# yashsmehta/visreps

Hardware: AMD Instinct MI355X
Metric: end-to-end RSA eval sec (extract→RDM→1000-bootstrap Spearman), N=10k stimuli (lower is better)
Workload: dtype bf16x3-split Gram, fp32 accumulate (|dSpearman| < 1e-5 vs fp64 RDMs: tests/test_benchsize.py) / exact int ranks, fp64 statistic

## Files before the change

### visreps_amd/csrc/rdm.hip

```cpp
#include <cstdlib>
#include <cstring>

#include "internal.h"

namespace vr {

typedef float f32x4 __attribute__((ext_vector_type(4)));
typedef float f32x16 __attribute__((ext_vector_type(16)));

constexpr int RSTAT_BS = 256;

__device__ inline double block_sum_f64(double v, double* lds) {
  for (int o = 32; o > 0; o >>= 1) v += __shfl_down(v, o, 64);
  const int lane = threadIdx.x & 63, wid = threadIdx.x >> 6;
  if (lane == 0) lds[wid] = v;
  __syncthreads();
  double s = 0;
  if (threadIdx.x == 0) {
    for (int w = 0; w < RSTAT_BS / 64; ++w) s += lds[w];
    lds[RSTAT_BS / 64] = s;
  }
  __syncthreads();
  s = lds[RSTAT_BS / 64];
  __syncthreads();
// ... 790 lines not shown
        aH[m] = __builtin_bit_cast(bf16x8, *reinterpret_cast<const u32x4*>(ar));
        aL[m] = __builtin_bit_cast(bf16x8, *reinterpret_cast<const u32x4*>(ar + 32));
      }
#pragma unroll
      for (int nn = 0; nn < 2; ++nn) {
        const uint16_t* br = Bs + (wc * 64 + nn * 32 + l32) * SROW + t * 16 + h * 8;
        bH[nn] = __builtin_bit_cast(bf16x8, *reinterpret_cast<const u32x4*>(br));
        bL[nn] = __builtin_bit_cast(bf16x8, *reinterpret_cast<const u32x4*>(br + 32));
      }
#pragma unroll
      for (int m = 0; m < 4; ++m)
#pragma unroll
        for (int nn = 0; nn < 2; ++nn)
          acc[m][nn] = __builtin_amdgcn_mfma_f32_32x32x16_bf16(aH[m], bH[nn], acc[m][nn], 0, 0, 0);
#pragma unroll
      for (int m = 0; m < 4; ++m)
#pragma unroll
        for (int nn = 0; nn < 2; ++nn)
          acc[m][nn] = __builtin_amdgcn_mfma_f32_32x32x16_bf16(aH[m], bL[nn], acc[m][nn], 0, 0, 0);
#pragma unroll
      for (int m = 0; m < 4; ++m)
#pragma unroll
        for (int nn = 0; nn < 2; ++nn)
          acc[m][nn] = __builtin_amdgcn_mfma_f32_32x32x16_bf16(aL[m], bH[nn], acc[m][nn], 0, 0, 0);
    }
    if (more) {
      uint16_t* nxt = lds + (cur ^ 1) * 2 * W_STAGE;
      store_rec_w(nxt, ga);
      if (!diag) store_rec_w(nxt + W_STAGE, gb);
    }
    if (P.flush && more && (kt + 1) % P.flush == 0) {
      gram_flush<WT>(acc, P.fbuf + (size_t)blockIdx.x * WT * WT, wr * 128, wc * 64, kt + 1 == P.flush);
    }
    __syncthreads();
  }
  if (P.flush && ns > P.flush) gram_unflush<WT>(acc, P.fbuf + (size_t)blockIdx.x * WT * WT, wr * 128, wc * 64);
  gram_store_w(P, acc, row0, col0, diag);
}

constexpr int P_PANEL = WT * 64;
constexpr int P_SLOT = 2 * P_PANEL;
constexpr int P_SLOTS = 4;
constexpr int P_AHEAD = P_SLOTS - 1;
static_assert(P_AHEAD == 3, "the counted waits of gram3p_step / gram3p_loop assume 4 slots");

__device__ inline void p_issue(const GramParams& P, char* panel, int64_t row0, int q) {
  const int lane = threadIdx.x & 63, wid = threadIdx.x >> 6;
  const int64_t st = q >> 1;
  const int t = q & 1;
#pragma unroll
  for (int i = 0; i < 2; ++i) {
    const int rbase = (wid * 2 + i) * 16;
    const int r = rbase + (lane >> 2);
    const int j = (lane & 3) ^ ((r >> 2) & 3);
    const int off = ((j & 2) << 5) + 32 * t + ((j & 1) << 4);
    const char* src = reinterpret_cast<const char*>(P.planes) + ((row0 + r) * P.nstage + st) * 128 + off;
    __builtin_amdgcn_global_load_lds(src, panel + rbase * 64, 16, 0, 0);
  }
}

__device__ inline bf16x8 p_frag(const char* panel, int row, int j) {
  return __builtin_bit_cast(bf16x8, *reinterpret_cast<const u32x4*>(panel + row * 64 + ((j ^ ((row >> 2) & 3)) << 4)));
}

template <int N>
__device__ inline void p_wait() {
  asm volatile("s_waitcnt vmcnt(%0)" ::"n"(N) : "memory");
}

struct PFrag {
  bf16x8 aH[4], aL[4], bH[2], bL[2];
};

__device__ inline void p_read(const char* As, const char* Bs, PFrag& f) {
  const int lane = threadIdx.x & 63, wid = threadIdx.x >> 6;
  const int wr = wid >> 2, wc = wid & 3, h = lane >> 5, l32 = lane & 31;
#pragma unroll
  for (int m = 0; m < 4; ++m) {
    const int r = wr * 128 + m * 32 + l32;
    f.aH[m] = p_frag(As, r, h);
    f.aL[m] = p_frag(As, r, 2 + h);
  }
#pragma unroll
  for (int nn = 0; nn < 2; ++nn) {
    const int r = wc * 64 + nn * 32 + l32;
    f.bH[nn] = p_frag(Bs, r, h);
    f.bL[nn] = p_frag(Bs, r, 2 + h);
  }
}

__device__ inline void p_mfma(const PFrag& f, f32x16 (&acc)[4][2]) {
#pragma unroll
  for (int m = 0; m < 4; ++m)
#pragma unroll
    for (int nn = 0; nn < 2; ++nn)
      acc[m][nn] = __builtin_amdgcn_mfma_f32_32x32x16_bf16(f.aH[m], f.bH[nn], acc[m][nn], 0, 0, 0);
#pragma unroll
  for (int m = 0; m < 4; ++m)
#pragma unroll
    for (int nn = 0; nn < 2; ++nn)
      acc[m][nn] = __builtin_amdgcn_mfma_f32_32x32x16_bf16(f.aH[m], f.bL[nn], acc[m][nn], 0, 0, 0);
#pragma unroll
  for (int m = 0; m < 4; ++m)
#pragma unroll
    for (int nn = 0; nn < 2; ++nn)
      acc[m][nn] = __builtin_amdgcn_mfma_f32_32x32x16_bf16(f.aL[m], f.bH[nn], acc[m][nn], 0, 0, 0);
}

template <bool DIAG>
__device__ inline void gram3p_step(const GramParams& P, char* lds, int64_t row0, int64_t col0, int q, int Q,
                                   const PFrag& cur, PFrag& nxt, f32x16 (&acc)[4][2]) {
  constexpr int PER = DIAG ? 2 : 4;
  if (q + 1 < Q) {
    const int left = Q - 2 - q;
    if (left >= 1)
      p_wait<PER>();
    else
      p_wait<0>();
    __builtin_amdgcn_s_barrier();
    if (q + P_AHEAD < Q) {
      char* slot = lds + ((q + P_AHEAD) % P_SLOTS) * P_SLOT;
      p_issue(P, slot, row0, q + P_AHEAD);
      if (!DIAG) p_issue(P, slot + P_PANEL, col0, q + P_AHEAD);
    }
    const char* As = lds + ((q + 1) % P_SLOTS) * P_SLOT;
    p_read(As, DIAG ? As : As + P_PANEL, nxt);
  }
  p_mfma(cur, acc);
  if (P.flush && (q & 1) && q + 1 < Q && ((q >> 1) + 1) % P.flush == 0) {
    const int wid = threadIdx.x >> 6;
    gram_flush<WT>(acc, P.fbuf + (size_t)blockIdx.x * WT * WT, (wid >> 2) * 128, (wid & 3) * 64,
                   (q >> 1) + 1 == P.flush);
  }
}

template <bool DIAG>
__device__ inline void gram3p_loop(const GramParams& P, char* lds, int64_t row0, int64_t col0, int ns,
                                   f32x16 (&acc)[4][2]) {
  const int Q = 2 * ns;
  constexpr int PER = DIAG ? 2 : 4;
  for (int q = 0; q < P_AHEAD && q < Q; ++q) {
    char* slot = lds + q * P_SLOT;
    p_issue(P, slot, row0, q);
    if (!DIAG) p_issue(P, slot + P_PANEL, col0, q);
  }
  if (Q > 2)
    p_wait<2 * PER>();
  else if (Q > 1)
    p_wait<PER>();
  else
    p_wait<0>();
  __builtin_amdgcn_s_barrier();
  PFrag f0, f1;
  p_read(lds, DIAG ? lds : lds + P_PANEL, f0);
  for (int q = 0; q < Q; q += 2) {
    gram3p_step<DIAG>(P, lds, row0, col0, q, Q, f0, f1, acc);
    gram3p_step<DIAG>(P, lds, row0, col0, q + 1, Q, f1, f0, acc);
  }
}

__device__ inline void gram_partial_w(const GramParams& P, f32x16 (&acc)[4][2], int split, int ltile) {
  const int lane = threadIdx.x & 63, wid = threadIdx.x >> 6;
  const int wr = wid >> 2, wc = wid & 3, h = lane >> 5, l32 = lane & 31;
  float* out = P.partial + ((int64_t)split * P.tile_count + ltile) * (WT * WT);
#pragma unroll
  for (int m = 0; m < 4; ++m)
#pragma unroll
    for (int nn = 0; nn < 2; ++nn) {
      const int lj = wc * 64 + nn * 32 + l32;
#pragma unroll
      for (int r = 0; r < 16; ++r) {
        const int li = wr * 128 + m * 32 + (r & 3) + 8 * (r >> 2) + 4 * h;
        out[li * WT + lj] = acc[m][nn][r];
      }
    }
}

__global__ __launch_bounds__(W_THREADS, 1) void k_gram3p(GramParams P) {
  __shared__ __attribute__((aligned(16))) char lds[P_SLOTS * P_SLOT];
  const int id = P.blk0 + (int)xcd_remap(blockIdx.x, (uint32_t)gridDim.x);
  const int split = id / P.tile_count, ltile = id % P.tile_count;
  int bi, bj;
  band_tile(ltile, P.tile0, P.tile_count, P.T, bi, bj);
  const bool diag = (bi == bj);
  const int64_t row0 = (int64_t)bi * WT, col0 = (int64_t)bj * WT;
  const int lane = threadIdx.x & 63, wid = threadIdx.x >> 6;
  const int wr = wid >> 2, wc = wid & 3;
  (void)lane;
  const int64_t sper = P.kslice / GK;
  const int64_t st0 = (int64_t)split * sper;
  const int ns = (int)(P.nstage - st0 < sper ? P.nstage - st0 : sper);
  GramParams S = P;
  S.planes = P.planes + st0 * 64;
  f32x16 acc[4][2];
#pragma unroll
  for (int a = 0; a < 4; ++a)
#pragma unroll
    for (int b = 0; b < 2; ++b)
#pragma unroll
      for (int e = 0; e < 16; ++e) acc[a][b][e] = 0.f;
  if (diag)
    gram3p_loop<true>(S, lds, row0, col0, ns, acc);
  else
    gram3p_loop<false>(S, lds, row0, col0, ns, acc);
  if (P.flush && ns > P.flush)
    gram_unflush<WT>(acc, P.fbuf + (size_t)blockIdx.x * WT * WT, wr * 128, wc * 64);
  if (P.splits == 1)
    gram_store_w(P, acc, row0, col0, diag);
  else
    gram_partial_w(P, acc, split, ltile);
}

__global__ __launch_bounds__(256) void k_gram_reduce_w(GramParams P) {
  __shared__ float tr[32][33];
  const int ltile = blockIdx.x;
  int bi, bj;
  band_tile(ltile, P.tile0, P.tile_count, P.T, bi, bj);
  const bool diag = (bi == bj);
  const int64_t row0 = (int64_t)bi * WT, col0 = (int64_t)bj * WT;
  const int tx = threadIdx.x & 31, ty = threadIdx.x >> 5;
  const int si0 = blockIdx.y * 32;
  for (int sj0 = 0; sj0 < WT; sj0 += 32) {
    for (int yy = ty; yy < 32; yy += 8) {
      const int li = si0 + yy, lj = sj0 + tx;
      const int pi = (diag && li > lj) ? lj : li, pj = (diag && li > lj) ? li : lj;
      float g = 0.f;
      for (int s = 0; s < P.splits; ++s)
        g += P.partial[((int64_t)s * P.tile_count + ltile) * (WT * WT) + pi * WT + pj];
      const int64_t i = row0 + li, j = col0 + lj;
      const float sI = (i < P.n) ? P.stdv[i] : 1.f, sJ = (j < P.n) ? P.stdv[j] : 1.f;
      const float v = rdm_value(g, i, j, P, sI, sJ);
      if (i < P.n && j < P.n) P.rdm[i * P.ldr + j] = v;
      tr[yy][tx] = v;
    }
    __syncthreads();
    if (!diag) {
      for (int yy = ty; yy < 32; yy += 8) {
        const int64_t j = col0 + sj0 + yy, i = row0 + si0 + tx;
        if (i < P.n && j < P.n) P.rdm[j * P.ldr + i] = tr[tx][yy];
      }
    }
    __syncthreads();
  }
}

constexpr int E_HALF = 128 * 128;
constexpr int E_STAGE = 4 * E_HALF;

__device__ inline uint32_t e_issue_off(const GramParams& P, int k) {
  const int lane = threadIdx.x & 63, wid = threadIdx.x >> 6;
  const int rr = wid * 16 + k * 8 + (lane >> 3);
  const int c = (lane & 7) ^ ((rr >> 1) & 7);
  return (uint32_t)rr * (uint32_t)P.nstage * 128u + (uint32_t)c * 16u;
}
__device__ inline void e_issue(const GramParams& P, char* sb, int h, int64_t row0, int64_t col0, int64_t st,
                               const uint32_t (&io)[2]) {
  const int wid = threadIdx.x >> 6;
  const int64_t rbase = (h < 2 ? row0 : col0) + (h & 1) * 128;
  const char* base = reinterpret_cast<const char*>(P.planes) + (rbase * P.nstage + st) * 128;
  char* half = sb + h * E_HALF;
#pragma unroll
  for (int k = 0; k < 2; ++k) {
    uint32_t off = io[k];
    asm volatile("" : "+v"(off));
    __builtin_amdgcn_global_load_lds(base + off, half + (wid * 16 + k * 8) * 128, 16, 0, 0);
  }
}

struct EFragA {
  bf16x8 hi[4], lo[4];
};
struct EFragB {
  bf16x8 hi[2], lo[2];
};

struct ELane {
  uint32_t hi, lo;
};
__device__ inline ELane e_lane() {
  const int lane = threadIdx.x & 63, g = lane >> 4, l16 = lane & 15, swz = (l16 >> 1) & 7;
  return ELane{(uint32_t)(l16 * 128 + ((g ^ swz) << 4)), (uint32_t)(l16 * 128 + (((4 + g) ^ swz) << 4))};
}
__device__ inline void e_read_a(const char* half, int r0, const ELane& o, EFragA& f) {
  uint32_t ohi = o.hi, olo = o.lo;
  asm volatile("" : "+v"(ohi), "+v"(olo));
#pragma unroll
  for (int m = 0; m < 4; ++m) {
    const char* row = half + (r0 + m * 16) * 128;
    f.hi[m] = __builtin_bit_cast(bf16x8, *reinterpret_cast<const u32x4*>(row + ohi));
    f.lo[m] = __builtin_bit_cast(bf16x8, *reinterpret_cast<const u32x4*>(row + olo));
  }
}
__device__ inline void e_read_b(const char* half, int r0, const ELane& o, EFragB& f) {
  uint32_t ohi = o.hi, olo = o.lo;
  asm volatile("" : "+v"(ohi), "+v"(olo));
#pragma unroll
  for (int n = 0; n < 2; ++n) {
    const char* row = half + (r0 + n * 16) * 128;
    f.hi[n] = __builtin_bit_cast(bf16x8, *reinterpret_cast<const u32x4*>(row + ohi));
    f.lo[n] = __builtin_bit_cast(bf16x8, *reinterpret_cast<const u32x4*>(row + olo));
  }
}

template <int MA, int NB, bool ONE>
__device__ inline void e_mfma(const EFragA& a, const EFragB& b, f32x4 (&acc)[8][4]) {
#pragma unroll
  for (int m = 0; m < 4; ++m)
#pragma unroll
    for (int n = 0; n < 2; ++n)
      acc[MA * 4 + m][NB * 2 + n] =
          __builtin_amdgcn_mfma_f32_16x16x32_bf16(a.hi[m], b.hi[n], acc[MA * 4 + m][NB * 2 + n], 0, 0, 0);
  if constexpr (ONE) {
#pragma unroll
    for (int m = 0; m < 4; ++m)
#pragma unroll
      for (int n = 0; n < 2; ++n)
        acc[MA * 4 + m][NB * 2 + n] =
            __builtin_amdgcn_mfma_f32_16x16x32_bf16(a.lo[m], b.lo[n], acc[MA * 4 + m][NB * 2 + n], 0, 0, 0);
    return;
  }
#pragma unroll
  for (int m = 0; m < 4; ++m)
#pragma unroll
    for (int n = 0; n < 2; ++n)
      acc[MA * 4 + m][NB * 2 + n] =
          __builtin_amdgcn_mfma_f32_16x16x32_bf16(a.hi[m], b.lo[n], acc[MA * 4 + m][NB * 2 + n], 0, 0, 0);
#pragma unroll
  for (int m = 0; m < 4; ++m)
#pragma unroll
    for (int n = 0; n < 2; ++n)
      acc[MA * 4 + m][NB * 2 + n] =
          __builtin_amdgcn_mfma_f32_16x16x32_bf16(a.lo[m], b.hi[n], acc[MA * 4 + m][NB * 2 + n], 0, 0, 0);
}

__device__ inline float* e_flush_base(float* buf) {
  const int lane = threadIdx.x & 63, wid = threadIdx.x >> 6;
  uint32_t off = (uint32_t)(((wid >> 2) * 128 + 4 * (lane >> 4)) * WT + (wid & 3) * 64 + (lane & 15));
  asm volatile("" : "+v"(off));
  return buf + off;
}
__device__ inline void e_flush(f32x4 (&acc)[8][4], float* buf, bool first) {
  float* b = e_flush_base(buf);
#pragma unroll
  for (int i = 0; i < 8; ++i)
#pragma unroll
    for (int j = 0; j < 4; ++j)
#pragma unroll
      for (int e = 0; e < 4; ++e) {
        float* p = b + (i * 16 + e) * WT + j * 16;
        *p = first ? acc[i][j][e] : *p + acc[i][j][e];
        acc[i][j][e] = 0.f;
      }
}
__device__ inline void e_unflush(f32x4 (&acc)[8][4], const float* buf) {
  const float* b = e_flush_base(const_cast<float*>(buf));
#pragma unroll
  for (int i = 0; i < 8; ++i)
#pragma unroll
    for (int j = 0; j < 4; ++j)
#pragma unroll
      for (int e = 0; e < 4; ++e) acc[i][j][e] += b[(i * 16 + e) * WT + j * 16];
}

template <bool ONE>
__device__ inline void e_store(const GramParams& P, f32x4 (&acc)[8][4], int64_t row0, int64_t col0, bool diag) {
  const int lane = threadIdx.x & 63, wid = threadIdx.x >> 6;
  const int wr = wid >> 2, wc = wid & 3, g = lane >> 4, l16 = lane & 15;
#pragma unroll
  for (int j4 = 0; j4 < 4; ++j4) {
    const int64_t j = col0 + wc * 64 + j4 * 16 + l16;
    const float sj = (j < P.n) ? P.stdv[j] : 1.f;
#pragma unroll
    for (int i8 = 0; i8 < 8; ++i8) {
      const int64_t ib = row0 + wr * 128 + i8 * 16 + 4 * g;
      float v[4];
#pragma unroll
      for (int e = 0; e < 4; ++e) {
        const int64_t i = ib + e;
        const float si = (i < P.n) ? P.stdv[i] : 1.f;
        v[e] = rdm_value_t<ONE>(acc[i8][j4][e], i, j, P, si, sj);
      }
      if (diag) {
#pragma unroll
        for (int e = 0; e < 4; ++e) {
          const int64_t i = ib + e;
          if (i <= j && j < P.n) {
            P.rdm[i * P.ldr + j] = v[e];
            if (i < j) P.rdm[j * P.ldr + i] = v[e];
          }
        }
        continue;
      }
#pragma unroll
      for (int e = 0; e < 4; ++e) {
        const int64_t i = ib + e;
        if (i < P.n && j < P.n) P.rdm[i * P.ldr + j] = v[e];
      }
      if (j < P.n) {
        float* dst = P.rdm + j * P.ldr + ib;
        if (P.vec && ib + 3 < P.n && ((P.ldr & 3) == 0)) {
          f32x4 w = {v[0], v[1], v[2], v[3]};
          *reinterpret_cast<f32x4*>(dst) = w;
        } else {
#pragma unroll
          for (int e = 0; e < 4; ++e)
            if (ib + e < P.n) dst[e] = v[e];
        }
      }
    }
  }
}

__device__ inline void e_barrier() {
  __builtin_amdgcn_s_barrier();
  asm volatile("" ::: "memory");
}

template <bool DIAG, bool ODD, bool ONE>
__device__ inline void e_stage(const GramParams& P, char* lds, int64_t row0, int64_t col0, int t, int ns,
                               const ELane& o, const uint32_t (&io)[2], EFragA& AX, EFragA& AY,
                               EFragB& BP, EFragB& BQ, f32x4 (&acc)[8][4]) {
  const int wid = threadIdx.x >> 6;
  const int wr = wid >> 2, wc = wid & 3;
  EFragB& B0 = ODD ? BQ : BP;
  EFragB& B1 = ODD ? BP : BQ;
  char* cur = lds + (t & 1) * E_STAGE;
  char* nxt = lds + ((t + 1) & 1) * E_STAGE;
  const int ha = wr, hb = DIAG ? (wc >> 1) : 2 + (wc >> 1);
  const int rb = (wc & 1) * 64;
  const bool more1 = t + 1 < ns, more2 = t + 2 < ns;
  e_barrier();
  if (more1) e_issue(P, nxt, 1, row0, col0, t + 1, io);
  e_read_b(cur + hb * E_HALF, rb + 32, o, B1);
  e_mfma<0, 0, ONE>(AX, B0, acc);
  e_barrier();
  if (!DIAG && more1) e_issue(P, nxt, 3, row0, col0, t + 1, io);
  e_read_a(cur + ha * E_HALF, 64, o, AY);
  e_mfma<0, 1, ONE>(AX, B1, acc);
  if (more1) {
    if (DIAG)
      p_wait<0>();
    else
      p_wait<2>();
  }
  e_barrier();
  if (!DIAG && more2) e_issue(P, cur, 2, row0, col0, t + 2, io);
  if (more1) e_read_a(nxt + ha * E_HALF, 0, o, AX);
  e_mfma<1, 1, ONE>(AY, B1, acc);
  if (!DIAG && more1) {
    if (more2)
      p_wait<2>();
    else
      p_wait<0>();
  }
  e_barrier();
  if (more2) e_issue(P, cur, 0, row0, col0, t + 2, io);
  if (more1) e_read_b(nxt + hb * E_HALF, rb, o, B1);
  e_mfma<1, 0, ONE>(AY, B0, acc);
  if (P.flush && more1 && (t + 1) % P.flush == 0) e_flush(acc, P.fbuf + (size_t)blockIdx.x * WT * WT, t + 1 == P.flush);
}

template <bool DIAG, bool ONE>
__device__ inline void e_loop(const GramParams& P, char* lds, int64_t row0, int64_t col0, int ns,
                              f32x4 (&acc)[8][4]) {
  const int wid = threadIdx.x >> 6;
  const int wr = wid >> 2, wc = wid & 3;
  const int ha = wr, hb = DIAG ? (wc >> 1) : 2 + (wc >> 1), rb = (wc & 1) * 64;
  const uint32_t io[2] = {e_issue_off(P, 0), e_issue_off(P, 1)};
  e_issue(P, lds, 0, row0, col0, 0, io);
  e_issue(P, lds, 1, row0, col0, 0, io);
  if (!DIAG) {
    e_issue(P, lds, 2, row0, col0, 0, io);
    e_issue(P, lds, 3, row0, col0, 0, io);
  }
  if (ns > 1) {
    if (!DIAG) e_issue(P, lds + E_STAGE, 2, row0, col0, 1, io);
    e_issue(P, lds + E_STAGE, 0, row0, col0, 1, io);
    if (DIAG)
      p_wait<2>();
    else
      p_wait<4>();
  } else {
    p_wait<0>();
  }
  e_barrier();
  const ELane o = e_lane();
  EFragA AX, AY;
  EFragB BP, BQ;
  e_read_a(lds + ha * E_HALF, 0, o, AX);
  e_read_b(lds + hb * E_HALF, rb, o, BP);
  for (int t = 0; t < ns; t += 2) {
    e_stage<DIAG, false, ONE>(P, lds, row0, col0, t, ns, o, io, AX, AY, BP, BQ, acc);
    if (t + 1 < ns) e_stage<DIAG, true, ONE>(P, lds, row0, col0, t + 1, ns, o, io, AX, AY, BP, BQ, acc);
  }
}

__device__ inline void e_partial(const GramParams& P, f32x4 (&acc)[8][4], int split, int ltile) {
  const int lane = threadIdx.x & 63, wid = threadIdx.x >> 6;
  const int wr = wid >> 2, wc = wid & 3, g = lane >> 4, l16 = lane & 15;
  float* out = P.partial + ((int64_t)split * P.tile_count + ltile) * (WT * WT);
#pragma unroll
  for (int i = 0; i < 8; ++i)
#pragma unroll
    for (int j = 0; j < 4; ++j)
#pragma unroll
      for (int e = 0; e < 4; ++e) out[(wr * 128 + i * 16 + 4 * g + e) * WT + wc * 64 + j * 16 + l16] = acc[i][j][e];
}

template <bool ONE>
__global__ __launch_bounds__(W_THREADS, 1) void k_gram3e(GramParams P) {
  __shared__ __attribute__((aligned(16))) char lds[2 * E_STAGE];
  const int id = P.blk0 + (int)xcd_remap(blockIdx.x, (uint32_t)gridDim.x);
  const int split = id / P.tile_count, ltile = id % P.tile_count;
  int bi, bj;
  band_tile(ltile, P.tile0, P.tile_count, P.T, bi, bj);
  const bool diag = (bi == bj);
  const int64_t row0 = (int64_t)bi * WT, col0 = (int64_t)bj * WT;
  const int64_t sper = P.kslice / GK;
  const int64_t st0 = (int64_t)split * sper;
  const int ns = (int)(P.nstage - st0 < sper ? P.nstage - st0 : sper);
  GramParams S = P;
  S.planes = P.planes + st0 * 64;
  f32x4 acc[8][4];
#pragma unroll
  for (int i = 0; i < 8; ++i)
#pragma unroll
    for (int j = 0; j < 4; ++j) acc[i][j] = f32x4{0.f, 0.f, 0.f, 0.f};
  if (diag)
    e_loop<true, ONE>(S, lds, row0, col0, ns, acc);
  else
    e_loop<false, ONE>(S, lds, row0, col0, ns, acc);
  if (P.flush && ns > P.flush) e_unflush(acc, P.fbuf + (size_t)blockIdx.x * WT * WT);
  if (P.splits == 1)
    e_store<ONE>(P, acc, row0, col0, diag);
  else
    e_partial(P, acc, split, ltile);
}

static bool env_flag(const char* name, bool dflt) {
  const char* e = getenv(name);
  return e && *e ? strcmp(e, "0") != 0 : dflt;
}

static bool gram_phased() {
  const char* e = getenv("VISREPS_GRAM_KERNEL");
  return !(e && strcmp(e, "p") == 0);
}

static bool gram_pipe() {
  const char* e = getenv("VISREPS_GRAM_PIPE");
  return !(e && strcmp(e, "0") == 0);
}

__global__ __launch_bounds__(256) void k_gram_reduce(GramParams P) {
  __shared__ float tr[32][33];
  const int ltile = blockIdx.x;
  int bi, bj;
  band_tile(ltile, P.tile0, P.tile_count, P.T, bi, bj);
  const bool diag = (bi == bj);
  const int64_t row0 = (int64_t)bi * GT, col0 = (int64_t)bj * GT;
  const int tx = threadIdx.x & 31, ty = threadIdx.x >> 5;
  for (int sb = 0; sb < (GT / 32) * (GT / 32); ++sb) {
    const int si0 = (sb / (GT / 32)) * 32, sj0 = (sb % (GT / 32)) * 32;
    for (int yy = ty; yy < 32; yy += 8) {
      const int li = si0 + yy, lj = sj0 + tx;
      float g = 0.f;
      const int pi = (diag && li > lj) ? lj : li, pj = (diag && li > lj) ? li : lj;
      for (int s = 0; s < P.splits; ++s)
        g += P.partial[((int64_t)s * P.tile_count + ltile) * (GT * GT) + pi * GT + pj];
      const int64_t i = row0 + li, j = col0 + lj;
      const float sI = (i < P.n) ? P.stdv[i] : 1.f, sJ = (j < P.n) ? P.stdv[j] : 1.f;
      const float v = rdm_value(g, i, j, P, sI, sJ);
      if (i < P.n && j < P.n) P.rdm[i * P.ldr + j] = v;
      tr[yy][tx] = v;
    }
    __syncthreads();
    if (!diag) {
      for (int yy = ty; yy < 32; yy += 8) {
        const int64_t j = col0 + sj0 + yy, i = row0 + si0 + tx;
        if (i < P.n && j < P.n) P.rdm[j * P.ldr + i] = tr[tx][yy];
      }
    }
    __syncthreads();
  }
}

static int64_t gram_tiles(int64_t n) {
  const int64_t T = (n + GT - 1) / GT;
  return T * (T + 1) / 2;
}

static void gram_geometry(int64_t n, int64_t d, int64_t count, int& T, int& ntiles,
                          int& splits, int64_t& kslice, bool fit = false) {
  T = (int)((n + GT - 1) / GT);
  ntiles = T * (T + 1) / 2;
  const int64_t kt = (d + GK - 1) / GK;
  const int target = 2 * num_cus();
  int s = 1;
  if (count < target) {
    s = fit ? (int)std::max<int64_t>(1, target / count) : (int)((target + count - 1) / count);
    const int64_t maxs = std::max<int64_t>(1, kt / 4);
    if (s > maxs) s = (int)maxs;
  }
  const int64_t per = (kt + s - 1) / s;
  kslice = per * GK;
  splits = (int)((d + kslice - 1) / kslice);
  if (splits < 1) splits = 1;
}

static bool gram_split(int64_t n, int64_t d) {
  const char* e = getenv("VISREPS_GRAM");
  if (e && strcmp(e, "fp32") == 0) return false;
  if (e && strcmp(e, "split") == 0) return true;
  return (double)n * (double)n * (double)d >= 1e10;
}

static int gram_generation(int nblk) {
  int gen = 2 * num_cus();
  if (const char* e = getenv("VISREPS_GRAM_GEN")) {
    const int v = atoi(e);
    gen = v > 0 ? v : nblk;
  }
  return std::max(1, gen);
}

static int64_t gram_tail(int64_t count) {
  const int gen = 2 * num_cus();
  if (getenv("VISREPS_GRAM_GEN") || count <= gen) return 0;
  const int64_t tail = count % gen;
  return (tail > 0 && tail <= gen / 2) ? tail : 0;
}

static size_t range_partial(int64_t n, int64_t d, int64_t count, bool fit_one = false) {
  if (count <= 0) return 0;
  int T, ntiles, splits;
  int64_t kslice;
  if (fit_one && count < 2 * num_cus()) {
    gram_geometry(n, d, count, T, ntiles, splits, kslice, true);
    return splits > 1 ? (size_t)splits * count * GT * GT : 0;
  }
  const int64_t tail = gram_tail(count);
  gram_geometry(n, d, count - tail, T, ntiles, splits, kslice);
  size_t part = splits > 1 ? (size_t)splits * (count - tail) : 0;
  if (tail > 0) {
    gram_geometry(n, d, tail, T, ntiles, splits, kslice, true);
    if (splits > 1) part = std::max(part, (size_t)splits * tail);
  }
  return part * GT * GT;
}

static int64_t tri_start(int64_t r, int64_t T) { return r * T - r * (r - 1) / 2; }

static int gram_wide_rows(int64_t n, int64_t d, bool split3) {
  if (!split3) return 0;
  if (const char* e = getenv("VISREPS_GRAM_WIDE"))
    if (strcmp(e, "0") == 0) return 0;
  const int64_t T2 = (n + WT - 1) / WT, gen = num_cus();
  const int64_t full = (T2 * (T2 + 1) / 2) / gen * gen;
  if (full < gen) return 0;
  int64_t R = 0;
  while (R + 1 <= T2 && tri_start(R + 1, T2) <= full) ++R;
  (void)d;
  return (int)R;
}

struct RangePlan {
  bool wide = false;
  int64_t s0 = 0, s1 = 0;
  int64_t r0 = 0, r_count = 0;
  int r_splits = 1;
  int64_t rem0 = 0, rem_count = 0;
  bool rem_fit = false;
};

static int wide_rem_splits(int64_t count, int64_t nstage) {
  const int64_t gen = num_cus();
  if (count <= 0 || count >= gen) return 1;
  int64_t s = gen / count;
  s = std::min<int64_t>(s, std::max<int64_t>(1, nstage / 8));
  const int64_t per = (nstage + s - 1) / s;
  return (int)((nstage + per - 1) / per);
}

static RangePlan plan_range(int64_t n, int64_t d, int64_t t0, int64_t t1, bool split3) {
  RangePlan rp;
  const int64_t total = gram_tiles(n), T = (n + GT - 1) / GT, T2 = (n + WT - 1) / WT;
  const int R = gram_wide_rows(n, d, split3);
  rp.rem0 = t0;
  rp.rem_count = t1 - t0;
  if (R == 0 || t1 <= t0) return rp;
  int64_t r0 = -1, r1 = -1;
  for (int64_t r = 0; r <= R; ++r) {
    if (tri_start(2 * r, T) == t0) r0 = r;
    if (tri_start(2 * r, T) == t1) r1 = r;
  }
  if (r0 < 0 || (t1 != total && r1 < 0)) return rp;
  const int64_t trem = tri_start(2 * (int64_t)R, T);
  rp.wide = true;
  rp.s0 = tri_start(r0, T2);
  rp.s1 = t1 == total ? tri_start(R, T2) : tri_start(r1, T2);
  rp.rem_count = 0;
  static const bool wide_rem = !(getenv("VISREPS_GRAM_WIDE_REM") && strcmp(getenv("VISREPS_GRAM_WIDE_REM"), "0") == 0);
  if (t1 == total && !wide_rem) {
    rp.rem0 = trem;
    rp.rem_count = total - trem;
    rp.rem_fit = true;
  } else if (t1 == total) {
    rp.r0 = tri_start(R, T2);
    rp.r_count = T2 * (T2 + 1) / 2 - rp.r0;
    rp.r_splits = wide_rem_splits(rp.r_count, (d + GK - 1) / GK);
  }
  return rp;
}

static int gram_flush_stages() {
  int f = 256;
  if (const char* e = getenv("VISREPS_GRAM_FLUSH")) f = atoi(e);
  return f > 0 ? f : 0;
}
static size_t gram_fbuf_floats() {
  return std::max<size_t>((size_t)2 * num_cus() * GT * GT, (size_t)num_cus() * WT * WT);
}

static size_t gram_ws(int64_t n, int64_t d, int64_t t0, int64_t t1, bool split3, void* base, float** mean,
                      float** stdv, float** partial, uint16_t** planes, float** fbuf = nullptr,
                      bool own_planes = true, uint32_t** flag = nullptr) {
  const RangePlan rp = plan_range(n, d, t0, t1, split3);
  size_t part = range_partial(n, d, rp.rem_count, rp.rem_fit);
  if (rp.r_splits > 1) part = std::max(part, (size_t)rp.r_count * rp.r_splits * WT * WT);
  Carver c(base);
  float* m = c.take<float>((size_t)n);
  float* s = c.take<float>((size_t)n);
  float* p = part ? c.take<float>(part) : nullptr;
  const int64_t prow = (n + WT - 1) / WT * WT;
  uint16_t* pl = split3 && own_planes ? c.take<uint16_t>((size_t)prow * (size_t)((d + GK - 1) / GK) * 64)
                                      : nullptr;
  const bool flush = gram_flush_stages() > 0 && (d + GK - 1) / GK > gram_flush_stages();
  float* fb = flush ? c.take<float>(gram_fbuf_floats()) : nullptr;
  uint32_t* fl = c.take<uint32_t>(64);
  if (flag) *flag = fl;
  if (fbuf) *fbuf = fb;
  if (mean) *mean = m;
  if (stdv) *stdv = s;
  if (partial) *partial = p;
  if (planes) *planes = pl;
  return c.bytes();
}

}

using namespace vr;

extern "C" {

size_t vr_rdm_pearson_workspace(int64_t n, int64_t d) {
  if (n <= 0 || d <= 0) return 256;
  return gram_ws(n, d, 0, gram_tiles(n), gram_split(n, d), nullptr, nullptr, nullptr, nullptr, nullptr);
}

size_t vr_rdm_tiles_workspace(int64_t n, int64_t d, int64_t tile_begin, int64_t tile_end) {
  if (n <= 0 || d <= 0 || tile_end <= tile_begin) return 256;
  return gram_ws(n, d, tile_begin, tile_end, gram_split(n, d), nullptr, nullptr, nullptr, nullptr,
                 nullptr);
}

int64_t vr_rdm_tile_count(int64_t n) { return n > 0 ? gram_tiles(n) : 0; }

int64_t vr_rdm_wide_rows(int64_t n, int64_t d) {
  return n > 0 && d > 0 ? gram_wide_rows(n, d, gram_split(n, d)) : 0;
}

int vr_rdm_range_aligned(int64_t n, int64_t d, int64_t tile_begin, int64_t tile_end) {
  if (n <= 0 || d <= 0 || tile_begin < 0 || tile_end > gram_tiles(n) || tile_end < tile_begin) return 0;
  if (tile_begin == tile_end) return 1;
  if (tile_begin == 0 && tile_end == gram_tiles(n)) return 1;
  return plan_range(n, d, tile_begin, tile_end, gram_split(n, d)).wide ? 1 : 0;
}

int64_t vr_rdm_tile_cost(int64_t n, int64_t tile) {
  int T = (int)((n + GT - 1) / GT), bi, bj;
  int p = (int)tile, r = 0;
  while (r + 1 < T && (int64_t)(r + 1) * T - (int64_t)(r + 1) * r / 2 <= p) ++r;
  bi = r;
  bj = r + (p - (r * T - r * (r - 1) / 2));
  const int64_t h = std::min<int64_t>(GT, n - (int64_t)bi * GT), w = std::min<int64_t>(GT, n - (int64_t)bj * GT);
  return bi == bj ? h * (h + 1) / 2 : h * w;
}

int vr_rdm_tile_rect(int64_t n, int64_t tile, int64_t* row0, int64_t* col0, int64_t* rows,
                     int64_t* cols) {
  VR_REQUIRE(n > 0 && tile >= 0 && tile < gram_tiles(n), "vr_rdm_tile_rect: tile %lld of %lld",
             (long long)tile, (long long)(n > 0 ? gram_tiles(n) : 0));
  VR_REQUIRE(row0 && col0 && rows && cols, "vr_rdm_tile_rect: null output");
  const int T = (int)((n + GT - 1) / GT);
  int p = (int)tile, r = 0;
  while (r + 1 < T && (int64_t)(r + 1) * T - (int64_t)(r + 1) * r / 2 <= p) ++r;
  const int bi = r, bj = r + (p - (r * T - r * (r - 1) / 2));
  *row0 = (int64_t)bi * GT;
  *col0 = (int64_t)bj * GT;
  *rows = std::min<int64_t>(GT, n - *row0);
  *cols = std::min<int64_t>(GT, n - *col0);
  return VR_OK;
}

int vr_row_stats_f32(const float* X, int64_t n, int64_t d, int64_t ldx, float* mean,
                     float* stdv, float correction, void* stream) {
  VR_REQUIRE(n >= 0 && d > 0 && ldx >= d, "vr_row_stats_f32: bad shape n=%lld d=%lld ldx=%lld",
             (long long)n, (long long)d, (long long)ldx);
  if (n == 0) return VR_OK;
  VR_REQUIRE(X && mean && stdv, "vr_row_stats_f32: null pointer");
  VR_REQUIRE(n <= INT32_MAX, "vr_row_stats_f32: n too large");
  const int vec = ((reinterpret_cast<uintptr_t>(X) & 15) == 0) && ((ldx & 3) == 0);
  k_row_stats<float><<<(unsigned)n, RSTAT_BS, 0, as_stream(stream)>>>(X, d, ldx, mean, stdv,
                                                                       correction, vec);
  VR_CHECK_LAUNCH();
  return VR_OK;
}

static int row_stats_bf16(const uint16_t* X, int64_t n, int64_t d, int64_t ldx, float* mean,
                          float* stdv, float correction, hipStream_t st) {
  const int vec = ((reinterpret_cast<uintptr_t>(X) & 7) == 0) && ((ldx & 3) == 0);
  k_row_stats<uint16_t><<<(unsigned)n, RSTAT_BS, 0, st>>>(X, d, ldx, mean, stdv, correction, vec);
  VR_CHECK_LAUNCH();
  return VR_OK;
}

struct PreSplit {
  const uint16_t* planes = nullptr;
  const float* mean = nullptr;
  const float* stdv = nullptr;
};

static int rdm_launch(const void* Xv, int64_t n, int64_t d, int64_t ldx, float* rdm, int64_t ldr,
                      float correction, int64_t tile_begin, int64_t tile_end, void* ws,
                      size_t ws_bytes, void* stream, size_t need, bool raw = false, bool bf16 = false,
                      const PreSplit& pre = PreSplit{}) {
  const float* X = static_cast<const float*>(Xv);
  if (ws_bytes < need || ws == nullptr) {
    set_error("vr_rdm_pearson: workspace %zu < %zu", ws_bytes, need);
// ... 416 lines not shown
```

Measured before the change: 1.897.

## Skew half the waves' MFMA schedule across barriers in Gram kernel

Waves with threadIdx>=256 (second half of the 8-wave block) now run a skewed stage schedule that splits each MFMA group in half and defers the second half past the next barrier. LDS reads are issued between the halves, with an explicit lgkmcnt wait added. The goal is to keep the two wave groups out of phase so one group's MFMAs overlap the other's LDS reads and barrier waits, cutting matrix-core idle time. The cost is a duplicated code path per block, which adds code size and risks higher register pressure and schedule fragility, and the carried pending MFMA has to be drained before each flush and at the end.

```diff
diff --git a/visreps_amd/csrc/rdm.hip b/visreps_amd/csrc/rdm.hip
--- a/visreps_amd/csrc/rdm.hip
+++ b/visreps_amd/csrc/rdm.hip
@@ -1116,17 +1116,17 @@
   }
 }
 
-template <int MA, int NB, bool ONE>
+template <int MA, int NB, bool ONE, int M0 = 0, int M1 = 4>
 __device__ inline void e_mfma(const EFragA& a, const EFragB& b, f32x4 (&acc)[8][4]) {
 #pragma unroll
-  for (int m = 0; m < 4; ++m)
+  for (int m = M0; m < M1; ++m)
 #pragma unroll
     for (int n = 0; n < 2; ++n)
       acc[MA * 4 + m][NB * 2 + n] =
           __builtin_amdgcn_mfma_f32_16x16x32_bf16(a.hi[m], b.hi[n], acc[MA * 4 + m][NB * 2 + n], 0, 0, 0);
   if constexpr (ONE) {
 #pragma unroll
-    for (int m = 0; m < 4; ++m)
+    for (int m = M0; m < M1; ++m)
 #pragma unroll
       for (int n = 0; n < 2; ++n)
         acc[MA * 4 + m][NB * 2 + n] =
@@ -1134,13 +1134,13 @@
     return;
   }
 #pragma unroll
-  for (int m = 0; m < 4; ++m)
+  for (int m = M0; m < M1; ++m)
 #pragma unroll
     for (int n = 0; n < 2; ++n)
       acc[MA * 4 + m][NB * 2 + n] =
           __builtin_amdgcn_mfma_f32_16x16x32_bf16(a.hi[m], b.lo[n], acc[MA * 4 + m][NB * 2 + n], 0, 0, 0);
 #pragma unroll
-  for (int m = 0; m < 4; ++m)
+  for (int m = M0; m < M1; ++m)
 #pragma unroll
     for (int n = 0; n < 2; ++n)
       acc[MA * 4 + m][NB * 2 + n] =
@@ -1274,7 +1274,73 @@
   if (P.flush && more1 && (t + 1) % P.flush == 0) e_flush(acc, P.fbuf + (size_t)blockIdx.x * WT * WT, t + 1 == P.flush);
 }
 
-template <bool DIAG, bool ONE>
+__device__ inline void e_reads_done() {
+  __builtin_amdgcn_sched_barrier(0);
+  asm volatile("s_waitcnt lgkmcnt(0)" ::: "memory");
+}
+
+template <bool DIAG, bool ODD, bool ONE>
+__device__ inline void e_stage_skew(const GramParams& P, char* lds, int64_t row0, int64_t col0, int t, int ns,
+                                    const ELane& o, const uint32_t (&io)[2], EFragA& AX, EFragA& AY,
+                                    EFragB& BP, EFragB& BQ, f32x4 (&acc)[8][4], bool& pend) {
+  const int wid = threadIdx.x >> 6;
+  const int wr = wid >> 2, wc = wid & 3;
+  EFragB& B0 = ODD ? BQ : BP;
+  EFragB& B1 = ODD ? BP : BQ;
+  char* cur = lds + (t & 1) * E_STAGE;
+  char* nxt = lds + ((t + 1) & 1) * E_STAGE;
+  const int ha = wr, hb = DIAG ? (wc >> 1) : 2 + (wc >> 1);
+  const int rb = (wc & 1) * 64;
+  const bool more1 = t + 1 < ns, more2 = t + 2 < ns;
+  e_barrier();
+  if (pend) e_mfma<1, 0, ONE, 2, 4>(AY, B1, acc);
+  __builtin_amdgcn_sched_barrier(0);
+  if (more1) e_issue(P, nxt, 1, row0, col0, t + 1, io);
+  e_read_b(cur + hb * E_HALF, rb + 32, o, B1);
+  e_mfma<0, 0, ONE, 0, 2>(AX, B0, acc);
+  e_reads_done();
+  e_barrier();
+  e_mfma<0, 0, ONE, 2, 4>(AX, B0, acc);
+  __builtin_amdgcn_sched_barrier(0);
+  if (!DIAG && more1) e_issue(P, nxt, 3, row0, col0, t + 1, io);
+  e_read_a(cur + ha * E_HALF, 64, o, AY);
+  e_mfma<0, 1, ONE, 0, 2>(AX, B1, acc);
+  e_reads_done();
+  if (more1) {
+    if (DIAG)
+      p_wait<0>();
+    else
+      p_wait<2>();
+  }
+  e_barrier();
+  e_mfma<0, 1, ONE, 2, 4>(AX, B1, acc);
+  __builtin_amdgcn_sched_barrier(0);
+  if (!DIAG && more2) e_issue(P, cur, 2, row0, col0, t + 2, io);
+  if (more1) e_read_a(nxt + ha * E_HALF, 0, o, AX);
+  e_mfma<1, 1, ONE, 0, 2>(AY, B1, acc);
+  e_reads_done();
+  if (!DIAG && more1) {
+    if (more2)
+      p_wait<2>();
+    else
+      p_wait<0>();
+  }
+  e_barrier();
+  e_mfma<1, 1, ONE, 2, 4>(AY, B1, acc);
+  __builtin_amdgcn_sched_barrier(0);
+  if (more2) e_issue(P, cur, 0, row0, col0, t + 2, io);
+  if (more1) e_read_b(nxt + hb * E_HALF, rb, o, B1);
+  e_mfma<1, 0, ONE, 0, 2>(AY, B0, acc);
+  e_reads_done();
+  pend = true;
+  if (P.flush && more1 && (t + 1) % P.flush == 0) {
+    e_mfma<1, 0, ONE, 2, 4>(AY, B0, acc);
+    pend = false;
+    e_flush(acc, P.fbuf + (size_t)blockIdx.x * WT * WT, t + 1 == P.flush);
+  }
+}
+
+template <bool DIAG, bool ONE, bool SKEW>
 __device__ inline void e_loop(const GramParams& P, char* lds, int64_t row0, int64_t col0, int ns,
                               f32x4 (&acc)[8][4]) {
   const int wid = threadIdx.x >> 6;
@@ -1303,6 +1369,21 @@
   EFragB BP, BQ;
   e_read_a(lds + ha * E_HALF, 0, o, AX);
   e_read_b(lds + hb * E_HALF, rb, o, BP);
+  if constexpr (SKEW) {
+    bool pend = false;
+    for (int t = 0; t < ns; t += 2) {
+      e_stage_skew<DIAG, false, ONE>(P, lds, row0, col0, t, ns, o, io, AX, AY, BP, BQ, acc, pend);
+      if (t + 1 < ns)
+        e_stage_skew<DIAG, true, ONE>(P, lds, row0, col0, t + 1, ns, o, io, AX, AY, BP, BQ, acc, pend);
+    }
+    if (pend) {
+      if (ns & 1)
+        e_mfma<1, 0, ONE, 2, 4>(AY, BP, acc);
+      else
+        e_mfma<1, 0, ONE, 2, 4>(AY, BQ, acc);
+    }
+    return;
+  }
   for (int t = 0; t < ns; t += 2) {
     e_stage<DIAG, false, ONE>(P, lds, row0, col0, t, ns, o, io, AX, AY, BP, BQ, acc);
     if (t + 1 < ns) e_stage<DIAG, true, ONE>(P, lds, row0, col0, t + 1, ns, o, io, AX, AY, BP, BQ, acc);
@@ -1319,6 +1400,25 @@
     for (int j = 0; j < 4; ++j)
 #pragma unroll
       for (int e = 0; e < 4; ++e) out[(wr * 128 + i * 16 + 4 * g + e) * WT + wc * 64 + j * 16 + l16] = acc[i][j][e];
+}
+
+template <bool ONE, bool SKEW>
+__device__ inline void e_tile(const GramParams& P, const GramParams& S, char* lds, int64_t row0, int64_t col0,
+                              int ns, bool diag, int split, int ltile) {
+  f32x4 acc[8][4];
+#pragma unroll
+  for (int i = 0; i < 8; ++i)
+#pragma unroll
+    for (int j = 0; j < 4; ++j) acc[i][j] = f32x4{0.f, 0.f, 0.f, 0.f};
+  if (diag)
+    e_loop<true, ONE, SKEW>(S, lds, row0, col0, ns, acc);
+  else
+    e_loop<false, ONE, SKEW>(S, lds, row0, col0, ns, acc);
+  if (P.flush && ns > P.flush) e_unflush(acc, P.fbuf + (size_t)blockIdx.x * WT * WT);
+  if (P.splits == 1)
+    e_store<ONE>(P, acc, row0, col0, diag);
+  else
+    e_partial(P, acc, split, ltile);
 }
 
 template <bool ONE>
@@ -1335,20 +1435,10 @@
   const int ns = (int)(P.nstage - st0 < sper ? P.nstage - st0 : sper);
   GramParams S = P;
   S.planes = P.planes + st0 * 64;
-  f32x4 acc[8][4];
-#pragma unroll
-  for (int i = 0; i < 8; ++i)
-#pragma unroll
-    for (int j = 0; j < 4; ++j) acc[i][j] = f32x4{0.f, 0.f, 0.f, 0.f};
-  if (diag)
-    e_loop<true, ONE>(S, lds, row0, col0, ns, acc);
+  if (__builtin_amdgcn_readfirstlane((int)threadIdx.x >> 8))
+    e_tile<ONE, true>(P, S, lds, row0, col0, ns, diag, split, ltile);
   else
-    e_loop<false, ONE>(S, lds, row0, col0, ns, acc);
-  if (P.flush && ns > P.flush) e_unflush(acc, P.fbuf + (size_t)blockIdx.x * WT * WT);
-  if (P.splits == 1)
-    e_store<ONE>(P, acc, row0, col0, diag);
-  else
-    e_partial(P, acc, split, ltile);
+    e_tile<ONE, false>(P, S, lds, row0, col0, ns, diag, split, ltile);
 }
 
 static bool env_flag(const char* name, bool dflt) {
```

After: 1.875 (median of 6 runs). -1.2%, faster.
